# wenxuanliu/multimodal-vae

Hardware: AMD Instinct MI355X
Metric: ELBO-steps/sec (whole node), MultiMNIST b=256 per GPU (higher is better)
Workload: dtype bf16; 1 GPU; multimnist_50x50_conv_mmvae_gru_text_3pass_elbo_step; batch_per_gpu=256, global_batch=256, n_latents=100, parallelism=dp1, hip_graph=False, optimizer=adam, mfma=bf16 in / fp32 acc; fp32 master weights, BN stats, PoE/KL/BCE/NLL, Adam

## Files before the change

### multimodal-vae_amd/csrc/convres.hip

```cpp
#include "gemm.h"
#include "convres_geo.h"
#include "convres.h"
#include "bn_dev.h"
#include "convres_epi.h"
#include <type_traits>
#include <cstdlib>

namespace {


template <int I, int N, typename F>
__device__ __forceinline__ void static_for(F&& f) {
    if constexpr (I < N) {
        f(std::integral_constant<int, I>{});
        static_for<I + 1, N>(f);
    }
}

struct ConvResArgs {
    const bf16* A;
    int nimg, group_n;
    const bf16* Wp[4];
    int Kpad[4];
    int Npad;
    bf16* out;
    int ldo;
    float2* colstats;
    const bf16* d_r;
    const float2* d_affine;
    const float2* d_meanrstd;
    float2* d_red;
    int dbg;
    BnFinalizeArgs fin;
    const bf16* t_r;
    const float2* t_red;
    const float2* t_mr;
    const float* t_gamma;
    float* t_dgamma; float* t_dbeta;
    float t_inv_cnt;
    int t_groups;
    bf16* stage_out;
    unsigned long long* ts;
};

constexpr unsigned OOB_OFF = 0x40000000u;

template <class G, int NI>
constexpr int tab_base(int c) {
    int r = 0;
    for (int i = 0; i < c; ++i) r += crgeo::cdiv(NI * G::OYX(i), 32) * 32;
    return r;
}

template <class G, int NI, int CH, int WAVES, int NG, bool SCR_OWN, int NSPLIT = 1, int KSPL = 1>
struct CrLayout {
    static constexpr int NTHR = WAVES * 64;
    static constexpr int MG = WAVES / (NG * KSPL), NT = G::N / 32 / NSPLIT / NG;
    static constexpr int max_mt() { int m = 0; for (int c = 0; c < G::NCLS; ++c) m = crgeo::cmax(m, crgeo::cdiv(crgeo::cdiv(NI * G::OYX(c), 32), MG)); return m; }
    static constexpr int RED_BYTES = KSPL > 1 ? WAVES * max_mt() * NT * 4096 : 0;
    static constexpr bool BDIR = CH == 0;
    static constexpr int BP = (CH * 16 + 8) * 2;
    static constexpr int W_BYTES = BDIR ? 0 : G::N * BP;
    static_assert(!BDIR || SCR_OWN, "direct-B kernels have no weight buffer to lend to the epilogue");
    static constexpr int IMG_ALL = NI * G::IMG_BYTES;
    static constexpr int TAB_BYTES = tab_base<G, NI>(G::NCLS) * 4;
    static constexpr int SCR_PITCH = 80, SCR_BYTES = 32 * SCR_PITCH;
    static constexpr int TRT_BYTES = G::C * 16;
    static constexpr int OFF_W = IMG_ALL, OFF_TAB = OFF_W + W_BYTES, OFF_TRT = OFF_TAB + TAB_BYTES,
                         OFF_SCR = OFF_TRT + TRT_BYTES, OFF_RED = OFF_SCR + (SCR_OWN ? WAVES * SCR_BYTES : 0), TOTAL = OFF_RED + RED_BYTES;
    static_assert((NSPLIT == 1 && KSPL == 1) || BDIR, "column / k splits exist for the direct-B kernels only");
    static_assert(G::N % (32 * NSPLIT * NG) == 0 && WAVES % (NG * KSPL) == 0, "wave decomposition");
    static_assert(SCR_OWN || W_BYTES >= WAVES * SCR_BYTES, "the weight buffer doubles as the epilogue scratch");
    static_assert(TOTAL <= 160 * 1024, "LDS budget");
};

template <class G, int NI, int CH, int WAVES, int NG, bool SCR_OWN, int MODE, int TR, int NSPLIT = 1, int KSPL = 1>
__global__ __launch_bounds__(WAVES * 64) void convres_kernel(const ConvResArgs a) {
    using L = CrLayout<G, NI, CH, WAVES, NG, SCR_OWN, NSPLIT, KSPL>;
    constexpr int NT = L::NT, MG = L::MG, NTHR = WAVES * 64;
    constexpr int BP = L::BP, SCR_PITCH = L::SCR_PITCH;
    extern __shared__ __attribute__((aligned(16))) char smem[];
    char* const img_s = smem;
    char* const w_s = smem + L::OFF_W;
    unsigned* const tab = reinterpret_cast<unsigned*>(smem + L::OFF_TAB);
    float4* const trt = reinterpret_cast<float4*>(smem + L::OFF_TRT);

    const int tid = threadIdx.x, lane = tid & 63;
    const int wave = __builtin_amdgcn_readfirstlane(tid >> 6);
    const int r = lane & 31, h = lane >> 5;
    const int kg = wave % KSPL, ng = (wave / KSPL) % NG, mg = wave / (KSPL * NG);
    const int ntb = blockIdx.y * (G::N / 32 / NSPLIT) + ng * NT;
    const int img0 = blockIdx.x * NI;
    const int grp = img0 / a.group_n;
    auto stamp = [&](int idx) {
        if (a.ts && lane == 0) a.ts[((size_t)blockIdx.x * WAVES + wave) * 16 + idx] = __builtin_amdgcn_s_memrealtime();
    };
    stamp(0);

    constexpr bool BDIR = L::BDIR;
    constexpr int WV = BDIR ? 1 : crgeo::cdiv(G::N * CH * 2, NTHR);
    i32x4c wreg[WV];
    auto w_fetch = [&](auto ci, auto chi) {
        constexpr int c = decltype(ci)::value, ch = decltype(chi)::value;
        constexpr int CHK = crgeo::cmin(CH, G::KSTEPS(c) - ch * CH), VPR = CHK * 2 + (BDIR ? 1 : 0), NV = G::N * VPR;
        const bf16* wsrc = a.Wp[c] + ch * CH * 16;
        const int kpad = a.Kpad[c];
#pragma unroll
        for (int it = 0; it < crgeo::cdiv(NV, NTHR); ++it) {
            const int v = tid + it * NTHR;
            const int n = v / VPR, kv = v - n * VPR;
            if (v < NV) wreg[it] = *reinterpret_cast<const i32x4c*>(wsrc + (size_t)n * kpad + kv * 8);
        }
    };
    auto w_store = [&](auto ci, auto chi) {
        constexpr int c = decltype(ci)::value, ch = decltype(chi)::value;
        constexpr int CHK = crgeo::cmin(CH, G::KSTEPS(c) - ch * CH), VPR = CHK * 2 + (BDIR ? 1 : 0), NV = G::N * VPR;
#pragma unroll
        for (int it = 0; it < crgeo::cdiv(NV, NTHR); ++it) {
            const int v = tid + it * NTHR;
            const int n = v / VPR, kv = v - n * VPR;
            if (v < NV) *reinterpret_cast<i32x4c*>(w_s + n * BP + kv * 16) = wreg[it];
        }
    };
    if constexpr (!BDIR) w_fetch(std::integral_constant<int, 0>{}, std::integral_constant<int, 0>{});

    constexpr int VPP = G::C / 8;
    constexpr int NVI = NI * G::AH * G::AW * VPP;
    constexpr int IT = crgeo::cdiv(NVI, NTHR), SB = 4, NB = crgeo::cdiv(IT, SB);
    static_assert(NTHR % VPP == 0, "a thread keeps its channel vector across staging iterations");
    const bf16* const src = a.A + (size_t)img0 * (G::AH * G::AW * G::C);
    const bf16* const src_r = TR == 2 ? a.t_r + (size_t)img0 * (G::AH * G::AW * G::C) : nullptr;
    bf16* const stage_dst = (TR != 0 && a.stage_out && blockIdx.y == 0) ? a.stage_out + (size_t)img0 * (G::AH * G::AW * G::C) : nullptr;
    i32x4c ireg[SB], rreg[TR == 2 ? SB : 1];
    auto i_fetch = [&](int b) {
#pragma unroll
        for (int i = 0; i < SB; ++i) {
            const int v = tid + (b * SB + i) * NTHR;
            if (b * SB + i < IT && v < NVI) {
                ireg[i] = *reinterpret_cast<const i32x4c*>(src + (size_t)v * 8);
                if constexpr (TR == 2) rreg[i] = *reinterpret_cast<const i32x4c*>(src_r + (size_t)v * 8);
            }
        }
    };
    float tc0[TR ? 8 : 1], tc1[TR ? 8 : 1], tc2[TR == 2 ? 8 : 1];
    auto i_store = [&](int b) {
#pragma unroll
        for (int i = 0; i < SB; ++i) {
            const int v = tid + (b * SB + i) * NTHR;
            if (b * SB + i < IT && v < NVI) {
                const int pix = v / VPP, cv = v - pix * VPP;
                const int img = pix / (G::AH * G::AW), p2 = pix - img * (G::AH * G::AW);
                const int iy = p2 / G::AW, ix = p2 - iy * G::AW;
                const int cell = G::cell(iy, ix);
                i32x4c val = ireg[i];
                if constexpr (TR == 1) {
                    const bf16x8 x = __builtin_bit_cast(bf16x8, val);
                    bf16x8 o;
#pragma unroll
                    for (int j = 0; j < 8; ++j) o[j] = (bf16)swish_fast((float)x[j] * tc0[j] + tc1[j]);
                    val = __builtin_bit_cast(i32x4c, o);
                } else if constexpr (TR == 2) {
                    const bf16x8 x = __builtin_bit_cast(bf16x8, val), rr = __builtin_bit_cast(bf16x8, rreg[i]);
                    bf16x8 o;
#pragma unroll
                    for (int j = 0; j < 8; ++j) o[j] = (bf16)((float)x[j] * tc0[j] + ((float)rr[j] * tc1[j] + tc2[j]));
                    val = __builtin_bit_cast(i32x4c, o);
                }
                if (cell >= 0) *reinterpret_cast<i32x4c*>(img_s + img * G::IMG_BYTES + cell + cv * 16) = val;
                if constexpr (TR != 0)
                    if (stage_dst) *reinterpret_cast<i32x4c*>(stage_dst + (size_t)v * 8) = val;
            }
        }
    };
    if (!(a.dbg & 4)) i_fetch(0);

    {
        const i32x4c z = {0, 0, 0, 0};
        for (int i = tid * 16; i < L::IMG_ALL; i += NTHR * 16) *reinterpret_cast<i32x4c*>(img_s + i) = z;
        const unsigned img_out = (unsigned)(G::OH * G::OW) * (unsigned)a.ldo * 2u;
        static_for<0, G::NCLS>([&](auto ci) {
            constexpr int c = decltype(ci)::value;
            constexpr int ROWS = NI * G::OYX(c), T = crgeo::cdiv(ROWS, 32);
            for (int e = tid; e < T * 32; e += NTHR) {
                unsigned v = OOB_OFF;
                if (e < ROWS) {
                    const int img = e / G::OYX(c), q = e - img * G::OYX(c);
                    const int jy = q / G::OX(c), jx = q - jy * G::OX(c);
                    v = (unsigned)img * img_out + (unsigned)((G::out_y(c, jy) * G::OW + G::out_x(c, jx)) * a.ldo * 2);
                }
                tab[tab_base<G, NI>(c) + e] = v;
            }
        });
        if constexpr (TR == 1) {
            for (int ch = tid; ch < G::C; ch += NTHR) {
                float2 aff, mr;
                bn_channel_tables(a.fin, grp, ch, aff, mr);
                trt[ch] = make_float4(aff.x, aff.y, 0.f, 0.f);
            }
            if (blockIdx.x == 0 && blockIdx.y == 0) {
                for (int i = tid; i < a.fin.G * G::C; i += NTHR) {
                    float2 aff, mr;
                    bn_channel_tables(a.fin, i / G::C, i % G::C, aff, mr);
                    a.fin.affine[i] = aff; a.fin.meanrstd[i] = mr;
                }
                bn_running_update(a.fin, tid, NTHR);
            }
        } else if constexpr (TR == 2) {
            for (int ch = tid; ch < G::C; ch += NTHR) {
                float sx = 0.f, sy = 0.f;
                for (int q = 0; q < MMVAE_STAT_SLOTS; ++q) {
                    const float2 t = a.t_red[((size_t)grp * MMVAE_STAT_SLOTS + q) * G::C + ch];
                    sx += t.x; sy += t.y;
                }
                const float2 mr = a.t_mr[grp * G::C + ch];
                const float g = a.t_gamma[ch] * mr.y, m1 = sx * a.t_inv_cnt, m2 = sy * a.t_inv_cnt;
                const float cb = -g * m2 * mr.y;
                trt[ch] = make_float4(g, cb, -cb * mr.x - g * m1, 0.f);
            }
            if (blockIdx.x == 0 && blockIdx.y == 0 && (a.t_dgamma || a.t_dbeta)) {
                for (int ch = tid; ch < G::C; ch += NTHR) {
                    float tg = 0.f, tb = 0.f;
                    for (int gg = 0; gg < a.t_groups; ++gg)
                        for (int q = 0; q < MMVAE_STAT_SLOTS; ++q) {
                            const float2 t = a.t_red[((size_t)gg * MMVAE_STAT_SLOTS + q) * G::C + ch];
                            tb += t.x; tg += t.y;
                        }
                    if (a.t_dgamma) a.t_dgamma[ch] += tg;
                    if (a.t_dbeta) a.t_dbeta[ch] += tb;
                }
            }
        }
    }
    stamp(1);
    __syncthreads();
    stamp(2);
    if constexpr (TR != 0) {
        const int cv0 = (tid % VPP) * 8;
#pragma unroll
        for (int j = 0; j < 8; ++j) {
            const float4 t = trt[cv0 + j];
            tc0[j] = t.x; tc1[j] = t.y;
            if constexpr (TR == 2) tc2[j] = t.z;
        }
    }
    if (!(a.dbg & 4)) {
        i_store(0);
        for (int b = 1; b < NB; ++b) { i_fetch(b); i_store(b); }
    }
    if constexpr (!BDIR) w_store(std::integral_constant<int, 0>{}, std::integral_constant<int, 0>{});
    stamp(3);
    __syncthreads();
    stamp(4);

    const __amdgpu_buffer_rsrc_t orsrc = __builtin_amdgcn_make_buffer_rsrc(
        a.out, 0, (int)((size_t)a.nimg * G::OH * G::OW * a.ldo * 2), 0x00020000);
    const __amdgpu_buffer_rsrc_t rrsrc = __builtin_amdgcn_make_buffer_rsrc(
        const_cast<bf16*>(a.d_r ? a.d_r : a.out), 0, (int)((size_t)a.nimg * G::OH * G::OW * a.ldo * 2), 0x00020000);
    const unsigned wg_out = (unsigned)img0 * (unsigned)(G::OH * G::OW) * (unsigned)a.ldo * 2u;
    float dsc[NT], dsh[NT], dmean[NT], drstd[NT], s1[NT], s2[NT];
#pragma unroll
    for (int nt = 0; nt < NT; ++nt) {
        const int co = (ntb + nt) * 32 + r;
        dsc[nt] = 1.f; dsh[nt] = 0.f; dmean[nt] = 0.f; drstd[nt] = 0.f; s1[nt] = 0.f; s2[nt] = 0.f;
        if (MODE == 1 && a.d_affine) { const float2 t = a.d_affine[grp * G::N + co]; dsc[nt] = t.x; dsh[nt] = t.y; }
        if (MODE == 1 && a.d_meanrstd) { const float2 t = a.d_meanrstd[grp * G::N + co]; dmean[nt] = t.x; drstd[nt] = t.y; }
    }
    char* const scr = (SCR_OWN ? smem + L::OFF_SCR : w_s) + wave * L::SCR_BYTES;
    __amdgpu_buffer_rsrc_t wrsrc[BDIR ? G::NCLS : 1];
    if constexpr (BDIR) {
#pragma unroll
        for (int i = 0; i < G::NCLS; ++i)
            wrsrc[i] = __builtin_amdgcn_make_buffer_rsrc(const_cast<bf16*>(a.Wp[i]), 0, a.Npad * a.Kpad[i] * 2, 0x00020000);
    }

    static_for<0, G::NCLS>([&](auto ci) {
        constexpr int c = decltype(ci)::value;
        constexpr int ROWS = NI * G::OYX(c), T = crgeo::cdiv(ROWS, 32), MT = crgeo::cdiv(T, MG);
        constexpr int KS = G::KSTEPS(c), CHE = BDIR ? KS : CH, NCH = crgeo::cdiv(KS, CHE);
        constexpr int KSL = KS / KSPL;
        int abase[MT];
#pragma unroll
        for (int m = 0; m < MT; ++m) {
            const int t = mg + m * MG;
            int R = (t < T ? t : 0) * 32 + r;
            R = R < ROWS ? R : ROWS - 1;
            const int img = R / G::OYX(c), q = R - img * G::OYX(c);
            const int jy = q / G::OX(c), jx = q - jy * G::OX(c);
            abase[m] = img * G::IMG_BYTES + G::base0(c) + jy * G::row_stride(c) + jx * G::col_stride(c) + h * 16;
            if constexpr (KSPL > 1) {
                static_assert(G::TH(c) % KSPL == 0, "the k split is by tap row");
                constexpr int KSL_ = KS / KSPL;
                abase[m] += kg * (G::step_off(c, KSL_) - G::step_off(c, 0));
            }
        }
        f32x16 acc[MT][NT];
#pragma unroll
        for (int m = 0; m < MT; ++m)
#pragma unroll
            for (int nt = 0; nt < NT; ++nt)
#pragma unroll
                for (int j = 0; j < 16; ++j) acc[m][nt][j] = 0.f;
        const int wrow = ((ng * NT) * 32 + r) * BP + h * 16;

        if constexpr (BDIR) {
            constexpr int PD = KSL < 8 ? KSL : 8;
            static_assert(KSPL == 1 || KSL % 2 == 0, "a wave's k range starts on a 32-column block of the packed weights");
            unsigned voff[NT];
#pragma unroll
            for (int nt = 0; nt < NT; ++nt)
                voff[nt] = (unsigned)(((2 * (ntb + nt) + (r >> 4)) * (a.Kpad[c] >> 5) * 64 + h * 16 + (r & 15)) * 16) +
                           (unsigned)(kg * (KSL / 2) * 1024);
            auto bload = [&](auto ki, bf16x8 (&fb)[NT]) {
                constexpr int kk = decltype(ki)::value;
#pragma unroll
                for (int nt = 0; nt < NT; ++nt)
                    fb[nt] = __builtin_bit_cast(bf16x8, __builtin_amdgcn_raw_buffer_load_b128(wrsrc[c], (int)voff[nt], (kk >> 1) * 1024 + (kk & 1) * 512, 0));
            };
            auto aload = [&](auto ki, bf16x8 (&fa)[MT]) {
                constexpr int kk = decltype(ki)::value;
                constexpr int aoff = G::step_off(c, kk);
#pragma unroll
                for (int m = 0; m < MT; ++m) fa[m] = *reinterpret_cast<const bf16x8*>(img_s + abase[m] + aoff);
            };
            bf16x8 bq[PD][NT], af[MT];
            static_for<0, PD>([&](auto pi) { bload(pi, bq[decltype(pi)::value]); });
            aload(std::integral_constant<int, 0>{}, af);
            __builtin_amdgcn_sched_group_barrier(0x100, MT, 0);
            if (!(a.dbg & 2))
            static_for<0, KSL>([&](auto ki) {
                constexpr int kk = decltype(ki)::value;
                constexpr int KS = KSL;
                bf16x8 bcur[NT], an[MT];
#pragma unroll
                for (int nt = 0; nt < NT; ++nt) bcur[nt] = bq[kk % PD][nt];
                if constexpr (kk + PD < KS) bload(std::integral_constant<int, kk + PD>{}, bq[kk % PD]);
                if constexpr (kk + 1 < KS) aload(std::integral_constant<int, kk + 1>{}, an);
#pragma unroll
                for (int m = 0; m < MT; ++m)
#pragma unroll
                    for (int nt = 0; nt < NT; ++nt)
                        acc[m][nt] = __builtin_amdgcn_mfma_f32_32x32x16_bf16(af[m], bcur[nt], acc[m][nt], 0, 0, 0);
                if constexpr (kk + PD < KS) __builtin_amdgcn_sched_group_barrier(0x020, NT, 0);
                if constexpr (kk + 1 < KS) __builtin_amdgcn_sched_group_barrier(0x100, MT, 0);
                __builtin_amdgcn_sched_group_barrier(0x008, MT * NT, 0);
                if constexpr (kk + 1 < KS) {
#pragma unroll
                    for (int m = 0; m < MT; ++m) af[m] = an[m];
                }
            });
            if constexpr (KSPL > 1) {
                float* const red = reinterpret_cast<float*>(smem + L::OFF_RED);
                constexpr int WSTR = L::max_mt() * NT * 1024;
#pragma unroll
                for (int m = 0; m < MT; ++m)
#pragma unroll
                    for (int nt = 0; nt < NT; ++nt)
#pragma unroll
                        for (int v4 = 0; v4 < 4; ++v4)
                            *reinterpret_cast<f32x4*>(red + wave * WSTR + ((m * NT + nt) * 64 + lane) * 16 + v4 * 4) =
                                f32x4{acc[m][nt][4 * v4], acc[m][nt][4 * v4 + 1], acc[m][nt][4 * v4 + 2], acc[m][nt][4 * v4 + 3]};
                __syncthreads();
                if (kg == 0) {
#pragma unroll
                    for (int k2 = 1; k2 < KSPL; ++k2)
#pragma unroll
                        for (int m = 0; m < MT; ++m)
#pragma unroll
                            for (int nt = 0; nt < NT; ++nt)
#pragma unroll
                                for (int v4 = 0; v4 < 4; ++v4) {
                                    const f32x4 t = *reinterpret_cast<const f32x4*>(red + (wave + k2) * WSTR + ((m * NT + nt) * 64 + lane) * 16 + v4 * 4);
                                    acc[m][nt][4 * v4] += t[0]; acc[m][nt][4 * v4 + 1] += t[1];
                                    acc[m][nt][4 * v4 + 2] += t[2]; acc[m][nt][4 * v4 + 3] += t[3];
                                }
                }
                __syncthreads();
            }
        }
        static_for<0, NCH>([&](auto chi) {
            constexpr int ch = decltype(chi)::value;
            constexpr int CHK = crgeo::cmin(CHE, KS - ch * CHE);
            constexpr bool last_chunk = ch + 1 == NCH;
            constexpr bool has_next = !BDIR && (!last_chunk || c + 1 < G::NCLS);
            constexpr int cn = last_chunk ? c + 1 : c, chn = last_chunk ? 0 : ch + 1;
            if constexpr (has_next) w_fetch(std::integral_constant<int, cn>{}, std::integral_constant<int, chn>{});
            if (!BDIR && !(a.dbg & 2)) {
                bf16x8 af[MT], bfr[NT];
                auto frag = [&](auto ki, bf16x8 (&fa)[MT], bf16x8 (&fb)[NT]) {
                    constexpr int kk = decltype(ki)::value;
                    constexpr int aoff = G::step_off(c, ch * CHE + kk);
#pragma unroll
                    for (int nt = 0; nt < NT; ++nt)
                        fb[nt] = *reinterpret_cast<const bf16x8*>(w_s + wrow + nt * 32 * BP + kk * 32);
#pragma unroll
                    for (int m = 0; m < MT; ++m) fa[m] = *reinterpret_cast<const bf16x8*>(img_s + abase[m] + aoff);
                };
                frag(std::integral_constant<int, 0>{}, af, bfr);
                __builtin_amdgcn_sched_group_barrier(0x100, MT + NT, 0);
                static_for<0, CHK>([&](auto ki) {
                    constexpr int kk = decltype(ki)::value;
                    bf16x8 an[MT], bn[NT];
                    if constexpr (kk + 1 < CHK) frag(std::integral_constant<int, kk + 1>{}, an, bn);
#pragma unroll
                    for (int m = 0; m < MT; ++m)
#pragma unroll
                        for (int nt = 0; nt < NT; ++nt)
                            acc[m][nt] = __builtin_amdgcn_mfma_f32_32x32x16_bf16(af[m], bfr[nt], acc[m][nt], 0, 0, 0);
                    if constexpr (kk + 1 < CHK) __builtin_amdgcn_sched_group_barrier(0x100, MT + NT, 0);
                    __builtin_amdgcn_sched_group_barrier(0x008, MT * NT, 0);
                    if constexpr (kk + 1 < CHK) {
#pragma unroll
                        for (int m = 0; m < MT; ++m) af[m] = an[m];
#pragma unroll
                        for (int nt = 0; nt < NT; ++nt) bfr[nt] = bn[nt];
                    }
                });
            }
            if constexpr (last_chunk) {
                stamp(5 + 2 * c);
                if constexpr (!SCR_OWN) __syncthreads();
#pragma unroll
                for (int m = 0; m < MT; ++m) {
                    const int t = mg + m * MG;
                    if (t < T && kg == 0) {
                        const unsigned* trow = tab + tab_base<G, NI>(c) + t * 32;
                        const unsigned off0 = trow[lane & 15], off1 = trow[16 + (lane & 15)];
                        const int rows_left = ROWS - t * 32;
#pragma unroll
                        for (int nt = 0; nt < NT; ++nt) {
                            const unsigned cob = (unsigned)(((ntb + nt) * 32 + (lane >> 4) * 8) * 2) + wg_out;
                            if (rows_left >= 32)
                                cr_epilogue_tile<MODE, false>(acc[m][nt], scr, lane, 32, off0 + cob, off1 + cob, orsrc, rrsrc,
                                                              dsc[nt], dsh[nt], dmean[nt], drstd[nt], s1[nt], s2[nt], !(a.dbg & 1));
                            else
                                cr_epilogue_tile<MODE, true>(acc[m][nt], scr, lane, rows_left, off0 + cob, off1 + cob, orsrc, rrsrc,
                                                             dsc[nt], dsh[nt], dmean[nt], drstd[nt], s1[nt], s2[nt], !(a.dbg & 1));
                        }
                    }
                }
            }
            if constexpr (last_chunk) stamp(6 + 2 * c);
            if constexpr (has_next) {
                __syncthreads();
                w_store(std::integral_constant<int, cn>{}, std::integral_constant<int, chn>{});
                __syncthreads();
            }
        });
    });

    stamp(13);
    float2* red = MODE == 1 ? a.d_red : a.colstats;
    if (red && kg == 0) {
        const int slot = (int)(blockIdx.x + wave) % MMVAE_STAT_SLOTS;
#pragma unroll
        for (int nt = 0; nt < NT; ++nt) {
            const float t1 = s1[nt] + __shfl_xor(s1[nt], 32, 64), t2 = s2[nt] + __shfl_xor(s2[nt], 32, 64);
            if (h == 0) {
                float2* d = red + ((size_t)grp * MMVAE_STAT_SLOTS + slot) * G::N + (ntb + nt) * 32 + r;
                atomicAdd(&d->x, t1);
                atomicAdd(&d->y, t2);
            }
        }
    }
    stamp(14);
}

}

namespace {

template <class G>
bool geo_matches(const GemmParams& p) {
    const GatherCommon& c = p.c;
    if (c.C != G::C || c.Ald != G::C || c.N != G::N || c.AH != G::AH || c.AW != G::AW || c.OH != G::OH || c.OW != G::OW) return false;
    if (c.nclasses != G::NCLS) return false;
    if (G::FORM == 0) {
        if (c.sy != G::S || c.sx != G::S || c.dy != 1 || c.dx != 1 || c.osy != 1 || c.osx != 1) return false;
    } else {
        if (c.sy != 1 || c.sx != 1 || c.dy != -1 || c.dx != -1 || c.osy != G::S || c.osx != G::S) return false;
    }
    for (int i = 0; i < G::NCLS; ++i) {
        const GatherClass& k = p.cls[i];
        if (k.OY != G::OY(i) || k.OX != G::OX(i) || k.TH != G::TH(i) || k.TW != G::TW(i) || k.offy != G::offy(i) ||
            k.offx != G::offx(i) || k.ooy != G::ph(i) || k.oox != G::pw(i) || k.K != G::K(i) || k.Kpad < G::K(i))
            return false;
    }
    return true;
}

template <class G, int NI, int CH, int WAVES, int NG, bool SCR_OWN, int MODE, int TR, int NSPLIT, int KSPL>
int launch_cr_mode(const ConvResArgs& a, hipStream_t stream) {
    using L = CrLayout<G, NI, CH, WAVES, NG, SCR_OWN, NSPLIT, KSPL>;
    static std::atomic<unsigned> attr_set{0};
    if (mmvae_first_use_on_device(attr_set))
        hipFuncSetAttribute(reinterpret_cast<const void*>(&convres_kernel<G, NI, CH, WAVES, NG, SCR_OWN, MODE, TR, NSPLIT, KSPL>),
                            hipFuncAttributeMaxDynamicSharedMemorySize, 160 * 1024);
    MMVAE_LAUNCH((convres_kernel<G, NI, CH, WAVES, NG, SCR_OWN, MODE, TR, NSPLIT, KSPL>), dim3(a.nimg / NI, NSPLIT), dim3(WAVES * 64), L::TOTAL, stream, a);
    MMVAE_TRY(mmvae_check_launch("convres"));
    return 1;
}

template <class G, int NI, int CH, int WAVES, int NG, bool SCR_OWN, int NSPLIT = 1, int KSPL = 1>
int launch_cr(const GemmParams& p, hipStream_t stream) {
    const GatherCommon& c = p.c;
    const int nimg = c.groups * c.group_n;
    ConvResArgs a{};
    a.A = c.A; a.nimg = nimg; a.group_n = c.group_n;
    constexpr bool BDIR = CH == 0;
    for (int i = 0; i < G::NCLS; ++i) {
        a.Wp[i] = BDIR ? p.cls[i].Wf : p.cls[i].Wp; a.Kpad[i] = p.cls[i].Kpad;
        if (BDIR && (!a.Wp[i] || a.Kpad[i] % 32 != 0)) return 0;
    }
    a.Npad = p.npad;
    a.out = p.out_bf; a.ldo = p.ldo; a.colstats = p.colstats;
    a.dbg = mmvae_knob("convres_dbg", 0);
    a.ts = reinterpret_cast<unsigned long long*>(((unsigned long long)(unsigned)mmvae_knob("convres_ts_hi", 0) << 32) |
                                                 (unsigned)mmvae_knob("convres_ts_lo", 0));
    a.d_r = p.d_r; a.d_affine = p.d_affine; a.d_meanrstd = p.d_meanrstd; a.d_red = p.d_red;
    const int kind = p.tr ? p.tr->kind : 0;
    MMVAE_REQUIRE(!(p.tr && p.tr->out == c.A) || NSPLIT == 1, "convres: an in-place staging by-product needs one workgroup per image tile");
    if (mmvae_probe_on()) {
        char tag[96];
        snprintf(tag, sizeof(tag), "convres form%d %d>%d %dx%d>%dx%d k%d s%d %s tr%d img%d", G::FORM, G::C, G::N, G::AH, G::AW, G::OH, G::OW,
                 G::KH, G::S, p.d_r ? "dgrad" : "fwd", kind, nimg);
        mmvae_probe_tag(tag, 2.0 * (G::FORM == 0 ? G::OH * G::OW : G::AH * G::AW) * G::KH * G::KW * G::C * G::N * (double)nimg);
    }
    if (kind == 1) {
        a.fin = p.tr->fin; a.stage_out = p.tr->out;
        MMVAE_REQUIRE(a.fin.C == G::C && a.fin.G == c.groups && a.fin.affine && a.fin.meanrstd && a.fin.gamma && a.fin.beta,
                      "convres: BatchNorm tables of the staged operand do not match the layer");
        MMVAE_REQUIRE(!p.d_r, "convres: forward-type staging transform on a data-gradient launch");
        return launch_cr_mode<G, NI, CH, WAVES, NG, SCR_OWN, 0, 1, NSPLIT, KSPL>(a, stream);
    }
    if (kind == 2) {
        const GatherTransform& t = *p.tr;
        MMVAE_REQUIRE(p.d_r && t.r && t.red && t.mr && t.gamma && t.groups == c.groups, "convres: BatchNorm-backward staging needs r / sums / tables");
        a.t_r = t.r; a.t_red = t.red; a.t_mr = t.mr; a.t_gamma = t.gamma; a.t_dgamma = t.dgamma; a.t_dbeta = t.dbeta;
        a.t_inv_cnt = t.inv_cnt; a.t_groups = t.groups; a.stage_out = t.out;
        return launch_cr_mode<G, NI, CH, WAVES, NG, SCR_OWN, 1, 2, NSPLIT, KSPL>(a, stream);
    }
    return p.d_r ? launch_cr_mode<G, NI, CH, WAVES, NG, SCR_OWN, 1, 0, NSPLIT, KSPL>(a, stream)
                 : launch_cr_mode<G, NI, CH, WAVES, NG, SCR_OWN, 0, 0, NSPLIT, KSPL>(a, stream);
}

bool features_ok(const GemmParams& p) {
    const GatherCommon& c = p.c;
    if (!p.out_bf || p.out_f || p.out_act_bf || p.e_mask || p.d_mask || p.d_colsum || p.d_cmod > 0 || p.d_bcast_n > 0) return false;
    if (c.a_bcast_n > 0 || c.a_mask || c.a_affine || c.a_act != ACT_NONE) return false;
    if (p.ldo != c.N || p.bias) return false;
    if (p.d_r && (p.d_ld != p.ldo || p.d_act != ACT_SWISH)) return false;
    if (p.colstats && p.d_r) return false;
    if ((size_t)c.groups * c.group_n * c.OH * c.OW * p.ldo * 2 >= (size_t)OOB_OFF) return false;
    return true;
}

template <class G, int NI, int CH, int WAVES, int NG, bool SCR_OWN, int NSPLIT = 1, int KSPL = 1>
int try_cr(const GemmParams& p, hipStream_t stream) {
    if (!geo_matches<G>(p)) return 0;
    if (p.c.group_n % NI != 0) return 0;
    return launch_cr<G, NI, CH, WAVES, NG, SCR_OWN, NSPLIT, KSPL>(p, stream);
}

using crgeo::Geo;
typedef Geo<0, 32, 64, 25, 25, 12, 12, 4, 4, 2, 1> G_mm_conv2;
typedef Geo<0, 64, 128, 12, 12, 6, 6, 4, 4, 2, 1> G_mm_conv3;
typedef Geo<1, 128, 64, 6, 6, 12, 12, 4, 4, 2, 1> G_mm_convT2;
typedef Geo<1, 64, 32, 12, 12, 25, 25, 5, 5, 2, 1> G_mm_convT3;
typedef Geo<1, 64, 32, 12, 12, 25, 25, 4, 4, 2, 1> G_mm_conv2d;
typedef Geo<0, 32, 64, 25, 25, 12, 12, 5, 5, 2, 1> G_mm_convT3d;
typedef Geo<1, 256, 128, 2, 2, 6, 6, 4, 4, 2, 0> G_mm_convT1;
typedef Geo<0, 128, 256, 6, 6, 2, 2, 4, 4, 2, 0> G_mm_conv4;
typedef Geo<0, 32, 64, 32, 32, 16, 16, 4, 4, 2, 1> G_ca_conv2;
typedef Geo<0, 64, 128, 16, 16, 8, 8, 4, 4, 2, 1> G_ca_conv3;
typedef Geo<1, 128, 64, 8, 8, 16, 16, 4, 4, 2, 1> G_ca_convT2;
typedef Geo<1, 64, 32, 16, 16, 32, 32, 4, 4, 2, 1> G_ca_convT3;

}

int try_launch_convres(const GemmParams& p, hipStream_t stream) {
    const bool forced = p.tr && p.tr->kind != 0;
    if ((!mmvae_knob("convres", 1) && !forced) || !features_ok(p)) {
        MMVAE_REQUIRE(!forced, "convres: a staging transform was requested for a launch this path does not cover");
        return 0;
    }
    int rc;
    const int nimg = p.c.groups * p.c.group_n;
    const int alt = mmvae_knob("convres_alt", 0);
    if ((rc = try_cr<G_mm_conv2, 1, 16, 8, 2, true>(p, stream)) != 0) return rc;
    if (alt != 3) {
        if ((rc = try_cr<G_mm_conv3, 2, 0, 8, 4, true>(p, stream)) != 0) return rc;
        if (nimg <= 256) { if ((rc = try_cr<G_mm_convT2, 2, 0, 8, 2, true>(p, stream)) != 0) return rc; }
        if ((rc = try_cr<G_mm_convT2, 4, 0, 8, 2, true>(p, stream)) != 0) return rc;
    }
    if ((rc = try_cr<G_mm_conv3, 2, 8, 8, 4, true>(p, stream)) != 0) return rc;
    if (nimg <= 256) { if ((rc = try_cr<G_mm_convT2, 2, 8, 4, 1, true>(p, stream)) != 0) return rc; }
    if ((rc = try_cr<G_mm_convT2, 4, 16, 8, 2, true>(p, stream)) != 0) return rc;
    if (alt == 1) { if ((rc = try_cr<G_mm_convT3, 4, 20, 8, 1, false>(p, stream)) != 0) return rc; }
    if ((rc = try_cr<G_mm_convT3, 2, 16, 4, 1, false>(p, stream)) != 0) return rc;
    if ((rc = try_cr<G_mm_conv2d, 1, 16, 8, 1, true>(p, stream)) != 0) return rc;
    if (alt != 4) {
        if (nimg > 256 && alt != 5) { if ((rc = try_cr<G_mm_convT1, 16, 0, 5, 1, true, 4, 1>(p, stream)) != 0) return rc; }
        if ((rc = try_cr<G_mm_convT1, 8, 0, 6, 1, true, 4, 2>(p, stream)) != 0) return rc;
        if ((rc = try_cr<G_mm_conv4, 8, 0, 8, 2, true, 4, 4>(p, stream)) != 0) return rc;
    }
    if ((rc = try_cr<G_mm_convT3d, 2, 10, 8, 2, false>(p, stream)) != 0) return rc;
    if (mmvae_knob("convres_celeba", 1)) {
        if ((rc = try_cr<G_ca_conv2, 1, 16, 8, 2, true>(p, stream)) != 0) return rc;
        if ((rc = try_cr<G_ca_conv3, 2, 0, 8, 4, true>(p, stream)) != 0) return rc;
        if ((rc = try_cr<G_ca_convT2, 4, 0, 8, 2, true>(p, stream)) != 0) return rc;
        if ((rc = try_cr<G_ca_convT3, 2, 16, 4, 1, false>(p, stream)) != 0) return rc;
    }
    MMVAE_REQUIRE(!forced, "convres: no kernel is compiled for the geometry of a launch with a staging transform");
    return 0;
}
```

### multimodal-vae_amd/csrc/convres_epi.h

```cpp
#pragma once
#include "common.h"

namespace {

typedef __attribute__((ext_vector_type(16))) float f32x16;
typedef __attribute__((ext_vector_type(4))) int i32x4c;

__device__ __forceinline__ float dswish_fast(float x) {
    const float s = __builtin_amdgcn_rcpf(1.0f + __expf(-x));
    return s * (1.0f + x * (1.0f - s));
}
__device__ __forceinline__ float swish_fast(float x) { return x * __builtin_amdgcn_rcpf(1.0f + __expf(-x)); }

typedef __attribute__((ext_vector_type(2))) float f32x2;
typedef __attribute__((address_space(3))) s16x4 lds_s16x4c;

template <int MODE, bool PARTIAL>
__device__ __forceinline__ void cr_epilogue_tile(const f32x16& acc, char* scr, int lane, int rows_valid, unsigned off0, unsigned off1,
                                                 __amdgpu_buffer_rsrc_t orsrc, __amdgpu_buffer_rsrc_t rrsrc, float dsc, float dsh,
                                                 float dmean, float drstd, float& s1, float& s2, bool store) {
    constexpr int SP = 80;
    const int r = lane & 31, h = lane >> 5, g = lane >> 4, i = lane & 15, q = i >> 2, p = i & 3;
    float v[16];
#pragma unroll
    for (int j = 0; j < 16; ++j) v[j] = acc[j];
    if constexpr (MODE == 1) {
        const i32x4c r0 = __builtin_bit_cast(i32x4c, __builtin_amdgcn_raw_buffer_load_b128(rrsrc, (int)off0, 0, 0));
        const i32x4c r1 = __builtin_bit_cast(i32x4c, __builtin_amdgcn_raw_buffer_load_b128(rrsrc, (int)off1, 0, 0));
        *reinterpret_cast<i32x4c*>(scr + i * SP + g * 16) = r0;
        *reinterpret_cast<i32x4c*>(scr + (16 + i) * SP + g * 16) = r1;
        asm volatile("" ::: "memory");
        const char* rb = scr + (4 * h + q) * SP + (16 * ((lane >> 4) & 1) + 4 * p) * 2;
        f32x2 t1 = {0.f, 0.f}, t2 = {0.f, 0.f};
#pragma unroll
        for (int k = 0; k < 4; ++k) {
            const bf16x4 rv = __builtin_bit_cast(bf16x4, __builtin_amdgcn_ds_read_tr16_b64_v4i16((lds_s16x4c*)(rb + 8 * k * SP)));
#pragma unroll
            for (int e = 0; e < 4; e += 2) {
                const f32x2 rr = {(float)rv[e], (float)rv[e + 1]};
                const f32x2 x = rr * dsc + dsh;
                f32x2 d = {dswish_fast(x[0]), dswish_fast(x[1])};
                f32x2 o = {v[4 * k + e], v[4 * k + e + 1]};
                o *= d;
                if constexpr (PARTIAL) {
                    const int row = 8 * k + 4 * h + e;
                    o[0] = row < rows_valid ? o[0] : 0.f;
                    o[1] = row + 1 < rows_valid ? o[1] : 0.f;
                }
                t1 += o;
                t2 += o * ((rr - dmean) * drstd);
                v[4 * k + e] = o[0]; v[4 * k + e + 1] = o[1];
            }
        }
        s1 += t1[0] + t1[1];
        s2 += t2[0] + t2[1];
        asm volatile("" ::: "memory");
    } else {
        f32x2 t1 = {0.f, 0.f}, t2 = {0.f, 0.f};
#pragma unroll
        for (int j = 0; j < 16; j += 2) {
            f32x2 o = {v[j], v[j + 1]};
            if constexpr (PARTIAL) {
                const int row = (j & 3) + 8 * (j >> 2) + 4 * h;
                o[0] = row < rows_valid ? o[0] : 0.f;
                o[1] = row + 1 < rows_valid ? o[1] : 0.f;
                v[j] = o[0]; v[j + 1] = o[1];
            }
            t1 += o;
            t2 += o * o;
        }
        s1 += t1[0] + t1[1];
        s2 += t2[0] + t2[1];
    }
#pragma unroll
    for (int k = 0; k < 4; ++k) {
        bf16x4 o;
#pragma unroll
        for (int e = 0; e < 4; ++e) o[e] = (bf16)v[4 * k + e];
        *reinterpret_cast<bf16x4*>(scr + r * SP + (8 * k + 4 * h) * 2) = o;
    }
    asm volatile("" ::: "memory");
    if (store) {
        const char* ob = scr + (8 * g + q) * SP + (4 * p) * 2;
        union { struct { s16x4 a, b; } s; i32x4c v; } u0, u1;
        u0.s.a = __builtin_amdgcn_ds_read_tr16_b64_v4i16((lds_s16x4c*)(ob));
        u0.s.b = __builtin_amdgcn_ds_read_tr16_b64_v4i16((lds_s16x4c*)(ob + 4 * SP));
        u1.s.a = __builtin_amdgcn_ds_read_tr16_b64_v4i16((lds_s16x4c*)(ob + 32));
        u1.s.b = __builtin_amdgcn_ds_read_tr16_b64_v4i16((lds_s16x4c*)(ob + 4 * SP + 32));
        __builtin_amdgcn_raw_buffer_store_b128(u0.v, orsrc, (int)off0, 0, 0);
        __builtin_amdgcn_raw_buffer_store_b128(u1.v, orsrc, (int)off1, 0, 0);
    }
    asm volatile("" ::: "memory");
}

}
```

Before: 1741 ELBO-steps/s.

## Prefetch weights, residual epilogue loads, and next staging batch ahead of use

Image staging now double-buffers its register sets, so the next batch's global loads are issued before the current batch is transformed and stored to LDS. Weight B-fragments for the first conv class are prefetched before the barrier, and for the next class at the end of each class loop. Residual (d_r) epilogue loads are issued during the final MFMA k-steps instead of inside the epilogue. The goal is to hide global-memory latency behind staging and MFMA work, at the cost of higher register pressure (up to 8×NT weight fragments plus MT×NT residual vectors), which could reduce occupancy or cause spills.

```diff
diff --git a/multimodal-vae_amd/csrc/convres.hip b/multimodal-vae_amd/csrc/convres.hip
--- a/multimodal-vae_amd/csrc/convres.hip
+++ b/multimodal-vae_amd/csrc/convres.hip
@@ -1,5 +1,6 @@
 #include "gemm.h"
 #include "convres_geo.h"
+#include "convres_stage.h"
 #include "convres.h"
 #include "bn_dev.h"
 #include "convres_epi.h"
@@ -124,35 +125,35 @@
     };
     if constexpr (!BDIR) w_fetch(std::integral_constant<int, 0>{}, std::integral_constant<int, 0>{});
 
-    constexpr int VPP = G::C / 8;
-    constexpr int NVI = NI * G::AH * G::AW * VPP;
-    constexpr int IT = crgeo::cdiv(NVI, NTHR), SB = 4, NB = crgeo::cdiv(IT, SB);
-    static_assert(NTHR % VPP == 0, "a thread keeps its channel vector across staging iterations");
+    using SG = crstage::Stage<G::C, NI * G::AH * G::AW, NTHR, TR == 2 ? 2 : 1>;
+    constexpr int VPP = SG::VPP, NVI = SG::NVI, SB = SG::SB, NB = SG::NB, AHEAD = SG::AHEAD;
     const bf16* const src = a.A + (size_t)img0 * (G::AH * G::AW * G::C);
     const bf16* const src_r = TR == 2 ? a.t_r + (size_t)img0 * (G::AH * G::AW * G::C) : nullptr;
     bf16* const stage_dst = (TR != 0 && a.stage_out && blockIdx.y == 0) ? a.stage_out + (size_t)img0 * (G::AH * G::AW * G::C) : nullptr;
-    i32x4c ireg[SB], rreg[TR == 2 ? SB : 1];
-    auto i_fetch = [&](int b) {
+    i32x4c ireg[AHEAD][SB], rreg[TR == 2 ? AHEAD : 1][TR == 2 ? SB : 1];
+    auto i_fetch = [&](auto bi) {
+        constexpr int b = decltype(bi)::value, s = SG::set(b);
 #pragma unroll
         for (int i = 0; i < SB; ++i) {
-            const int v = tid + (b * SB + i) * NTHR;
-            if (b * SB + i < IT && v < NVI) {
-                ireg[i] = *reinterpret_cast<const i32x4c*>(src + (size_t)v * 8);
-                if constexpr (TR == 2) rreg[i] = *reinterpret_cast<const i32x4c*>(src_r + (size_t)v * 8);
+            const int v = SG::vec(tid, b, i);
+            if (SG::live(b, i) && v < NVI) {
+                ireg[s][i] = *reinterpret_cast<const i32x4c*>(src + (size_t)v * 8);
+                if constexpr (TR == 2) rreg[s][i] = *reinterpret_cast<const i32x4c*>(src_r + (size_t)v * 8);
             }
         }
     };
     float tc0[TR ? 8 : 1], tc1[TR ? 8 : 1], tc2[TR == 2 ? 8 : 1];
-    auto i_store = [&](int b) {
+    auto i_store = [&](auto bi) {
+        constexpr int b = decltype(bi)::value, s = SG::set(b);
 #pragma unroll
         for (int i = 0; i < SB; ++i) {
-            const int v = tid + (b * SB + i) * NTHR;
-            if (b * SB + i < IT && v < NVI) {
+            const int v = SG::vec(tid, b, i);
+            if (SG::live(b, i) && v < NVI) {
                 const int pix = v / VPP, cv = v - pix * VPP;
                 const int img = pix / (G::AH * G::AW), p2 = pix - img * (G::AH * G::AW);
                 const int iy = p2 / G::AW, ix = p2 - iy * G::AW;
                 const int cell = G::cell(iy, ix);
-                i32x4c val = ireg[i];
+                i32x4c val = ireg[s][i];
                 if constexpr (TR == 1) {
                     const bf16x8 x = __builtin_bit_cast(bf16x8, val);
                     bf16x8 o;
@@ -160,7 +161,7 @@
                     for (int j = 0; j < 8; ++j) o[j] = (bf16)swish_fast((float)x[j] * tc0[j] + tc1[j]);
                     val = __builtin_bit_cast(i32x4c, o);
                 } else if constexpr (TR == 2) {
-                    const bf16x8 x = __builtin_bit_cast(bf16x8, val), rr = __builtin_bit_cast(bf16x8, rreg[i]);
+                    const bf16x8 x = __builtin_bit_cast(bf16x8, val), rr = __builtin_bit_cast(bf16x8, rreg[s][i]);
                     bf16x8 o;
 #pragma unroll
                     for (int j = 0; j < 8; ++j) o[j] = (bf16)((float)x[j] * tc0[j] + ((float)rr[j] * tc1[j] + tc2[j]));
@@ -172,7 +173,30 @@
             }
         }
     };
-    if (!(a.dbg & 4)) i_fetch(0);
+    if (!(a.dbg & 4)) i_fetch(std::integral_constant<int, 0>{});
+
+    __amdgpu_buffer_rsrc_t wrsrc[BDIR ? G::NCLS : 1];
+    if constexpr (BDIR) {
+#pragma unroll
+        for (int i = 0; i < G::NCLS; ++i)
+            wrsrc[i] = __builtin_amdgcn_make_buffer_rsrc(const_cast<bf16*>(a.Wp[i]), 0, a.Npad * a.Kpad[i] * 2, 0x00020000);
+    }
+    constexpr int PDMAX = 8;
+    bf16x8 bqn[BDIR ? PDMAX : 1][NT];
+    auto b_voff = [&](auto ci, int nt) {
+        constexpr int c = decltype(ci)::value, KSL = G::KSTEPS(c) / KSPL;
+        return (unsigned)(((2 * (ntb + nt) + (r >> 4)) * (a.Kpad[c] >> 5) * 64 + h * 16 + (r & 15)) * 16) + (unsigned)(kg * (KSL / 2) * 1024);
+    };
+    auto b_load = [&](auto ci, auto ki, bf16x8 (&fb)[NT]) {
+        constexpr int c = decltype(ci)::value, kk = decltype(ki)::value;
+#pragma unroll
+        for (int nt = 0; nt < NT; ++nt)
+            fb[nt] = __builtin_bit_cast(bf16x8, __builtin_amdgcn_raw_buffer_load_b128(wrsrc[c], (int)b_voff(ci, nt), (kk >> 1) * 1024 + (kk & 1) * 512, 0));
+    };
+    auto b_prefetch = [&](auto ci) {
+        constexpr int c = decltype(ci)::value, KSL = G::KSTEPS(c) / KSPL, PD = KSL < PDMAX ? KSL : PDMAX;
+        static_for<0, PD>([&](auto pi) { b_load(ci, pi, bqn[decltype(pi)::value]); });
+    };
 
     {
         const i32x4c z = {0, 0, 0, 0};
@@ -244,9 +268,13 @@
         }
     }
     if (!(a.dbg & 4)) {
-        i_store(0);
-        for (int b = 1; b < NB; ++b) { i_fetch(b); i_store(b); }
-    }
+        static_for<0, NB>([&](auto bi) {
+            constexpr int b = decltype(bi)::value;
+            if constexpr (b + 1 < NB) i_fetch(std::integral_constant<int, b + 1>{});
+            i_store(bi);
+        });
+    }
+    if constexpr (BDIR) b_prefetch(std::integral_constant<int, 0>{});
     if constexpr (!BDIR) w_store(std::integral_constant<int, 0>{}, std::integral_constant<int, 0>{});
     stamp(3);
     __syncthreads();
@@ -266,12 +294,6 @@
         if (MODE == 1 && a.d_meanrstd) { const float2 t = a.d_meanrstd[grp * G::N + co]; dmean[nt] = t.x; drstd[nt] = t.y; }
     }
     char* const scr = (SCR_OWN ? smem + L::OFF_SCR : w_s) + wave * L::SCR_BYTES;
-    __amdgpu_buffer_rsrc_t wrsrc[BDIR ? G::NCLS : 1];
-    if constexpr (BDIR) {
-#pragma unroll
-        for (int i = 0; i < G::NCLS; ++i)
-            wrsrc[i] = __builtin_amdgcn_make_buffer_rsrc(const_cast<bf16*>(a.Wp[i]), 0, a.Npad * a.Kpad[i] * 2, 0x00020000);
-    }
 
     static_for<0, G::NCLS>([&](auto ci) {
         constexpr int c = decltype(ci)::value;
@@ -301,21 +323,31 @@
 #pragma unroll
                 for (int j = 0; j < 16; ++j) acc[m][nt][j] = 0.f;
         const int wrow = ((ng * NT) * 32 + r) * BP + h * 16;
+        unsigned eo0[MT], eo1[MT];
+#pragma unroll
+        for (int m = 0; m < MT; ++m) {
+            const int t = mg + m * MG;
+            const bool mine = t < T && kg == 0;
+            const unsigned* trow = tab + tab_base<G, NI>(c) + (t < T ? t : 0) * 32;
+            eo0[m] = mine ? trow[lane & 15] : OOB_OFF; eo1[m] = mine ? trow[16 + (lane & 15)] : OOB_OFF;
+        }
+        i32x4c dr0[MT][NT], dr1[MT][NT];
+        auto dr_fetch = [&]() {
+            if constexpr (MODE == 1) {
+#pragma unroll
+                for (int m = 0; m < MT; ++m)
+#pragma unroll
+                    for (int nt = 0; nt < NT; ++nt) {
+                        const unsigned cob = (unsigned)(((ntb + nt) * 32 + (lane >> 4) * 8) * 2) + wg_out;
+                        cr_epilogue_fetch(rrsrc, eo0[m] + cob, eo1[m] + cob, dr0[m][nt], dr1[m][nt]);
+                    }
+            }
+        };
 
         if constexpr (BDIR) {
-            constexpr int PD = KSL < 8 ? KSL : 8;
+            constexpr int PD = KSL < PDMAX ? KSL : PDMAX;
             static_assert(KSPL == 1 || KSL % 2 == 0, "a wave's k range starts on a 32-column block of the packed weights");
-            unsigned voff[NT];
-#pragma unroll
-            for (int nt = 0; nt < NT; ++nt)
-                voff[nt] = (unsigned)(((2 * (ntb + nt) + (r >> 4)) * (a.Kpad[c] >> 5) * 64 + h * 16 + (r & 15)) * 16) +
-                           (unsigned)(kg * (KSL / 2) * 1024);
-            auto bload = [&](auto ki, bf16x8 (&fb)[NT]) {
-                constexpr int kk = decltype(ki)::value;
-#pragma unroll
-                for (int nt = 0; nt < NT; ++nt)
-                    fb[nt] = __builtin_bit_cast(bf16x8, __builtin_amdgcn_raw_buffer_load_b128(wrsrc[c], (int)voff[nt], (kk >> 1) * 1024 + (kk & 1) * 512, 0));
-            };
+            auto bload = [&](auto ki, bf16x8 (&fb)[NT]) { b_load(ci, ki, fb); };
             auto aload = [&](auto ki, bf16x8 (&fa)[MT]) {
                 constexpr int kk = decltype(ki)::value;
                 constexpr int aoff = G::step_off(c, kk);
@@ -323,7 +355,10 @@
                 for (int m = 0; m < MT; ++m) fa[m] = *reinterpret_cast<const bf16x8*>(img_s + abase[m] + aoff);
             };
             bf16x8 bq[PD][NT], af[MT];
-            static_for<0, PD>([&](auto pi) { bload(pi, bq[decltype(pi)::value]); });
+#pragma unroll
+            for (int p = 0; p < PD; ++p)
+#pragma unroll
+                for (int nt = 0; nt < NT; ++nt) bq[p][nt] = bqn[p][nt];
             aload(std::integral_constant<int, 0>{}, af);
             __builtin_amdgcn_sched_group_barrier(0x100, MT, 0);
             if (!(a.dbg & 2))
@@ -334,6 +369,7 @@
 #pragma unroll
                 for (int nt = 0; nt < NT; ++nt) bcur[nt] = bq[kk % PD][nt];
                 if constexpr (kk + PD < KS) bload(std::integral_constant<int, kk + PD>{}, bq[kk % PD]);
+                if constexpr (kk == (KS > PD ? KS - PD : 0)) dr_fetch();
                 if constexpr (kk + 1 < KS) aload(std::integral_constant<int, kk + 1>{}, an);
 #pragma unroll
                 for (int m = 0; m < MT; ++m)
@@ -341,6 +377,7 @@
                     for (int nt = 0; nt < NT; ++nt)
                         acc[m][nt] = __builtin_amdgcn_mfma_f32_32x32x16_bf16(af[m], bcur[nt], acc[m][nt], 0, 0, 0);
                 if constexpr (kk + PD < KS) __builtin_amdgcn_sched_group_barrier(0x020, NT, 0);
+                if constexpr (MODE == 1 && kk == (KS > PD ? KS - PD : 0)) __builtin_amdgcn_sched_group_barrier(0x020, 2 * MT * NT, 0);
                 if constexpr (kk + 1 < KS) __builtin_amdgcn_sched_group_barrier(0x100, MT, 0);
                 __builtin_amdgcn_sched_group_barrier(0x008, MT * NT, 0);
                 if constexpr (kk + 1 < KS) {
@@ -348,6 +385,8 @@
                     for (int m = 0; m < MT; ++m) af[m] = an[m];
                 }
             });
+            else dr_fetch();
+            if constexpr (c + 1 < G::NCLS) b_prefetch(std::integral_constant<int, c + 1>{});
             if constexpr (KSPL > 1) {
                 float* const red = reinterpret_cast<float*>(smem + L::OFF_RED);
                 constexpr int WSTR = L::max_mt() * NT * 1024;
@@ -384,6 +423,7 @@
             constexpr bool has_next = !BDIR && (!last_chunk || c + 1 < G::NCLS);
             constexpr int cn = last_chunk ? c + 1 : c, chn = last_chunk ? 0 : ch + 1;
             if constexpr (has_next) w_fetch(std::integral_constant<int, cn>{}, std::integral_constant<int, chn>{});
+            if constexpr (!BDIR && last_chunk) dr_fetch();
             if (!BDIR && !(a.dbg & 2)) {
                 bf16x8 af[MT], bfr[NT];
                 auto frag = [&](auto ki, bf16x8 (&fa)[MT], bf16x8 (&fb)[NT]) {
@@ -423,18 +463,17 @@
                 for (int m = 0; m < MT; ++m) {
                     const int t = mg + m * MG;
                     if (t < T && kg == 0) {
-                        const unsigned* trow = tab + tab_base<G, NI>(c) + t * 32;
-                        const unsigned off0 = trow[lane & 15], off1 = trow[16 + (lane & 15)];
+                        const unsigned off0 = eo0[m], off1 = eo1[m];
                         const int rows_left = ROWS - t * 32;
 #pragma unroll
                         for (int nt = 0; nt < NT; ++nt) {
                             const unsigned cob = (unsigned)(((ntb + nt) * 32 + (lane >> 4) * 8) * 2) + wg_out;
                             if (rows_left >= 32)
-                                cr_epilogue_tile<MODE, false>(acc[m][nt], scr, lane, 32, off0 + cob, off1 + cob, orsrc, rrsrc,
-                                                              dsc[nt], dsh[nt], dmean[nt], drstd[nt], s1[nt], s2[nt], !(a.dbg & 1));
+                                cr_epilogue_finish<MODE, false>(acc[m][nt], scr, lane, 32, off0 + cob, off1 + cob, orsrc, dr0[m][nt], dr1[m][nt],
+                                                                dsc[nt], dsh[nt], dmean[nt], drstd[nt], s1[nt], s2[nt], !(a.dbg & 1));
                             else
-                                cr_epilogue_tile<MODE, true>(acc[m][nt], scr, lane, rows_left, off0 + cob, off1 + cob, orsrc, rrsrc,
-                                                             dsc[nt], dsh[nt], dmean[nt], drstd[nt], s1[nt], s2[nt], !(a.dbg & 1));
+                                cr_epilogue_finish<MODE, true>(acc[m][nt], scr, lane, rows_left, off0 + cob, off1 + cob, orsrc, dr0[m][nt], dr1[m][nt],
+                                                               dsc[nt], dsh[nt], dmean[nt], drstd[nt], s1[nt], s2[nt], !(a.dbg & 1));
                         }
                     }
                 }
diff --git a/multimodal-vae_amd/csrc/convres_epi.h b/multimodal-vae_amd/csrc/convres_epi.h
--- a/multimodal-vae_amd/csrc/convres_epi.h
+++ b/multimodal-vae_amd/csrc/convres_epi.h
@@ -15,18 +15,21 @@
 typedef __attribute__((ext_vector_type(2))) float f32x2;
 typedef __attribute__((address_space(3))) s16x4 lds_s16x4c;
 
+__device__ __forceinline__ void cr_epilogue_fetch(__amdgpu_buffer_rsrc_t rrsrc, unsigned off0, unsigned off1, i32x4c& r0, i32x4c& r1) {
+    r0 = __builtin_bit_cast(i32x4c, __builtin_amdgcn_raw_buffer_load_b128(rrsrc, (int)off0, 0, 0));
+    r1 = __builtin_bit_cast(i32x4c, __builtin_amdgcn_raw_buffer_load_b128(rrsrc, (int)off1, 0, 0));
+}
+
 template <int MODE, bool PARTIAL>
-__device__ __forceinline__ void cr_epilogue_tile(const f32x16& acc, char* scr, int lane, int rows_valid, unsigned off0, unsigned off1,
-                                                 __amdgpu_buffer_rsrc_t orsrc, __amdgpu_buffer_rsrc_t rrsrc, float dsc, float dsh,
-                                                 float dmean, float drstd, float& s1, float& s2, bool store) {
+__device__ __forceinline__ void cr_epilogue_finish(const f32x16& acc, char* scr, int lane, int rows_valid, unsigned off0, unsigned off1,
+                                                   __amdgpu_buffer_rsrc_t orsrc, const i32x4c& r0, const i32x4c& r1, float dsc, float dsh,
+                                                   float dmean, float drstd, float& s1, float& s2, bool store) {
     constexpr int SP = 80;
     const int r = lane & 31, h = lane >> 5, g = lane >> 4, i = lane & 15, q = i >> 2, p = i & 3;
     float v[16];
 #pragma unroll
     for (int j = 0; j < 16; ++j) v[j] = acc[j];
     if constexpr (MODE == 1) {
-        const i32x4c r0 = __builtin_bit_cast(i32x4c, __builtin_amdgcn_raw_buffer_load_b128(rrsrc, (int)off0, 0, 0));
-        const i32x4c r1 = __builtin_bit_cast(i32x4c, __builtin_amdgcn_raw_buffer_load_b128(rrsrc, (int)off1, 0, 0));
         *reinterpret_cast<i32x4c*>(scr + i * SP + g * 16) = r0;
         *reinterpret_cast<i32x4c*>(scr + (16 + i) * SP + g * 16) = r1;
         asm volatile("" ::: "memory");
@@ -93,4 +96,13 @@
     asm volatile("" ::: "memory");
 }
 
+template <int MODE, bool PARTIAL>
+__device__ __forceinline__ void cr_epilogue_tile(const f32x16& acc, char* scr, int lane, int rows_valid, unsigned off0, unsigned off1,
+                                                 __amdgpu_buffer_rsrc_t orsrc, __amdgpu_buffer_rsrc_t rrsrc, float dsc, float dsh,
+                                                 float dmean, float drstd, float& s1, float& s2, bool store) {
+    i32x4c r0 = {0, 0, 0, 0}, r1 = {0, 0, 0, 0};
+    if constexpr (MODE == 1) cr_epilogue_fetch(rrsrc, off0, off1, r0, r1);
+    cr_epilogue_finish<MODE, PARTIAL>(acc, scr, lane, rows_valid, off0, off1, orsrc, r0, r1, dsc, dsh, dmean, drstd, s1, s2, store);
 }
+
+}
diff --git a/multimodal-vae_amd/csrc/convres_stage.h b/multimodal-vae_amd/csrc/convres_stage.h
--- /dev/null
+++ b/multimodal-vae_amd/csrc/convres_stage.h
@@ -0,0 +1,26 @@
+#pragma once
+
+namespace crstage {
+
+constexpr int cdiv(int a, int b) { return (a + b - 1) / b; }
+
+constexpr int SBATCH = 4;
+constexpr int MAXV = 16;
+
+template <int C, int NPIX, int NTHR, int NTENS>
+struct Stage {
+    static_assert(C % 8 == 0, "a vector is 8 channels");
+    static constexpr int VPP = C / 8;
+    static constexpr int NVI = NPIX * VPP;
+    static constexpr int IT = cdiv(NVI, NTHR);
+    static_assert(NTHR % VPP == 0, "a thread keeps its channel vector across staging iterations");
+    static constexpr int SB = SBATCH, NB = cdiv(IT, SB);
+    static constexpr int AHEAD = NB > 1 ? 2 : 1;
+    static_assert(AHEAD * SB * NTENS <= MAXV && NB * SB >= IT, "staging register budget");
+    static constexpr int iter(int b, int i) { return b * SB + i; }
+    static constexpr bool live(int b, int i) { return iter(b, i) < IT; }
+    static constexpr int vec(int tid, int b, int i) { return tid + iter(b, i) * NTHR; }
+    static constexpr int set(int b) { return b % AHEAD; }
+};
+
+}
```

Result: no change. 1758 ELBO-steps/s (median of 6 runs) (+0.9%).
